# KillingSpark/zstd-rs

Hardware: AMD Instinct MI355X
Metric: decompressed_GB_per_s (higher is better)
Workload: dtype u8

## Files before the change

### zstd-rs_amd/csrc/zg_engine.cpp

```cpp
#include "zg_engine.h"
#include <stdlib.h>
#include <algorithm>
#include <string.h>

namespace zg {

#define ZG_HIP(call)                                  \
  do {                                                \
    hipError_t e_ = (call);                           \
    if (e_ != hipSuccess) return eng->fail(e_, #call); \
  } while (0)

#ifdef ZG_DEV_SWITCHES
static int g_poison = -1;
static uint64_t g_poisoned = 0;
uint64_t Poison::scratch_cap = 0;
int Poison::value() { return g_poison; }
void Poison::set(int v) { g_poison = v; }
void Poison::fill(void* p, size_t n, hipStream_t s) {
  if (g_poison < 0 || !p || !n) return;
  if (hipMemsetAsync(p, g_poison, n, s) == hipSuccess) g_poisoned += n;
}
void Poison::fill_now(void* p, size_t n) {
  if (g_poison < 0 || !p || !n) return;
// ... 28 lines not shown
}

int SidePass::reserve(size_t bytes) {
  const int st = buf.reserve(bytes);
  if (st) return st;
  Poison::fill_now(buf.p, buf.cap);
  for (hipEvent_t& e : ev) if (!e && hipEventCreate(&e) != hipSuccess) return ZG_HIP_ERROR;
  return 0;
}
hipError_t SidePass::upload(const void* a, size_t ab, const void* b, size_t bb, hipStream_t s) const {
  const hipError_t e = hipMemcpyAsync(buf.p, a, ab, hipMemcpyHostToDevice, s);
  return e != hipSuccess || !bb ? e : hipMemcpyAsync(at<uint8_t>(ab), b, bb, hipMemcpyHostToDevice, s);
}
hipError_t SidePass::end(hipStream_t s) const {
  const hipError_t e = hipGetLastError();
  return e != hipSuccess ? e : hipEventRecord(ev[1], s);
}
static hipError_t us_between(hipEvent_t a, hipEvent_t b, uint64_t* us) {
  float ms = 0;
  const hipError_t e = hipEventElapsedTime(&ms, a, b);
  if (e == hipSuccess) *us = (uint64_t)(ms * 1000.0f + 0.5f);
  return e;
}
hipError_t SidePass::elapsed_us(uint64_t* us) const { return us_between(ev[0], ev[1], us); }
void SidePass::release(int device) {
  if (buf.p && device >= 0) (void)hipSetDevice(device);
  buf.release();
  for (hipEvent_t& e : ev) if (e) { (void)hipEventDestroy(e); e = nullptr; }
  n = 0;
}

int Scratch::init_events() {
  if (have_events) return 0;
  for (auto& e : ev)
    if (hipEventCreate(&e) != hipSuccess) return ZG_HIP_ERROR;
  for (auto& e : ev_huf)
    if (hipEventCreate(&e) != hipSuccess) return ZG_HIP_ERROR;
  if (hipEventCreateWithFlags(&ev_fork, hipEventDisableTiming) != hipSuccess) return ZG_HIP_ERROR;
  if (hipEventCreateWithFlags(&ev_fork3, hipEventDisableTiming) != hipSuccess) return ZG_HIP_ERROR;
  if (hipEventCreateWithFlags(&ev_up, hipEventDisableTiming) != hipSuccess) return ZG_HIP_ERROR;
  for (auto& e : ev_sw)
    if (hipEventCreateWithFlags(&e, hipEventDisableTiming) != hipSuccess) return ZG_HIP_ERROR;
  for (auto& e : ev_flat)
    if (hipEventCreateWithFlags(&e, hipEventDisableTiming) != hipSuccess) return ZG_HIP_ERROR;
  have_events = true;
  return 0;
}
void Scratch::release_but_output() {
  DevBuf* all[] = {&d_src, &d_aux, &d_fparsed, &d_slot_log, &d_fse, &d_huf, &d_hufmax, &d_lit, &d_seq, &d_og, &d_raw};
  for (DevBuf* b : all) b->release();
}
template <class F> void Scratch::each_buf(F f) {
  DevBuf* all[] = {&d_src, &d_blocks, &d_frames, &d_aux, &d_fparsed, &d_slot_log, &d_fse, &d_huf, &d_hufmax, &d_status, &d_lit, &d_seq, &d_seqout, &d_pos,
                   &d_frameout, &d_dst, &d_seqblocks, &d_hufitems, &d_hufgroups, &d_totals, &d_og, &d_units, &d_unitinfo, &d_stepunits, &d_swdesc,
                   &d_dbg, &d_raw, &d_unitlist};
  for (DevBuf* b : all) f(*b);
}
void Scratch::release() {
  each_buf([](DevBuf& b) { b.release(); });
  for (auto& e : ev)
    if (e) { (void)hipEventDestroy(e); e = nullptr; }
  for (auto& e : ev_huf)
    if (e) { (void)hipEventDestroy(e); e = nullptr; }
  if (ev_fork) { (void)hipEventDestroy(ev_fork); ev_fork = nullptr; }
  if (ev_fork3) { (void)hipEventDestroy(ev_fork3); ev_fork3 = nullptr; }
  if (ev_up) { (void)hipEventDestroy(ev_up); ev_up = nullptr; }
  for (auto& e : ev_sw)
    if (e) { (void)hipEventDestroy(e); e = nullptr; }
  for (auto& e : ev_flat)
    if (e) { (void)hipEventDestroy(e); e = nullptr; }
  have_events = false;
}

int Engine::fail(hipError_t e, const char* what) {
  last_error = std::string(what) + ": " + hipGetErrorString(e);
  return ZG_HIP_ERROR;
}

Tuning Tuning::from_env() {
  Tuning t;
#ifdef ZG_DEV_SWITCHES
  t.dev_build = true;
  auto num = [](const char* name, uint32_t* v, bool positive) { const char* e = getenv(name); if (e && atoi(e) >= (positive ? 1 : 0)) *v = (uint32_t)atoi(e); return e != nullptr && atoi(e) >= 0; };
  auto is0 = [](const char* name) { const char* e = getenv(name); return e && e[0] == '0'; };
  num("ZGPU_UNIT_BLOCKS", &t.unit_blocks, true);
  t.direct = !is0("ZGPU_DIRECT");
  num("ZGPU_RAMP", &t.ramp_percent, false);
  t.sparse_set = num("ZGPU_SPARSE_MAX", &t.sparse_max, false);
  if (is0("ZGPU_LIT_DIRECT")) t.lit_direct = 0;
  else { const char* e = getenv("ZGPU_LIT_DIRECT"); if (e && e[0] == '1') t.lit_direct = 1; }
  { uint32_t v = 0; if (num("ZGPU_DIRECT_SHARE", &v, true) && v >= 10) t.direct_share10 = v; }
  t.debug_timers = getenv("ZGPU_DEBUG_TIMERS") != nullptr;
  { const char* e = getenv("ZGPU_FORCE_INORDER"); t.force_inorder = e && e[0] == '1'; }
  num("ZGPU_FLAT_MODE", &t.flat_mode, false);
  num("ZGPU_SWEEP_W", &t.sweep_w, true);
  t.overlap = !is0("ZGPU_OVERLAP");
  t.no_sweep = getenv("ZGPU_DEBUG_NO_SWEEP") != nullptr;
  t.sweep_split = !is0("ZGPU_SWEEP_SPLIT");
  t.no_exact = getenv("ZGPU_DEBUG_NO_EXACT") != nullptr;
  t.no_presize = is0("ZGPU_PRESIZE");
  { uint32_t v = 0; if (num("ZGPU_FLAT4", &v, false)) t.flat4 = (int)v; }
  { uint32_t v = 0; if (num("ZGPU_SEQ_PACKED", &v, false)) t.seq_packed = (int)v; }
  { const char* e = getenv("ZGPU_FLAT_T"); t.flat_shape = (e && atoi(e) == 512) ? 1 : 0; }
  num("ZGPU_SWEEP_MODE", &t.sweep.mode, false);
  num("ZGPU_SWEEP_NB", &t.sweep.nbatch, true);
  num("ZGPU_SWEEP_GROUP", &t.sweep.group, true);
  num("ZGPU_SWEEP_HEAD_LDS", &t.sweep.head_lds, false);
  num("ZGPU_SWEEP_HEAD_NB", &t.sweep.head_nbatch, true);
  { const char* e = getenv("ZGPU_FRAMES_SUBMIT_BYTES"); if (e && atoll(e) > 0) t.frames_submit_bytes = (uint64_t)atoll(e); }
  { const char* e = getenv("ZGPU_MEASURE_SUBMIT_BYTES"); if (e && atoll(e) > 0) t.measure_submit_bytes = (uint64_t)atoll(e); }
  num("ZGPU_SCATTER_CHUNK", &t.scatter_chunk, true);
  { const char* e = getenv("ZGPU_POISON"); if (e && e[0] && atoi(e) >= 0 && atoi(e) <= 255) t.poison = atoi(e); }
// ... 485 lines not shown
  b->bb.seq_packed_force = tn.seq_packed;
  if (tn.direct_share10) b->bb.direct_share10 = tn.direct_share10;
  b->bb.finish();
  BatchBuilder& bb = b->bb;
  Scratch* sc = b->sc = acquire();
  Poison::begin_submit();
  const uint32_t nb = (uint32_t)bb.blocks.size(), nf = (uint32_t)bb.frames.size();
  auto up = [&](DevBuf& d, const void* h, size_t bytes) -> int {
    int st = d.reserve(bytes ? bytes : 16);
    if (st) return st;
    Poison::fill(d.p, d.cap, us);
    if (bytes && hipMemcpyAsync(d.p, h, bytes, hipMemcpyHostToDevice, us) != hipSuccess) return ZG_HIP_ERROR;
    return 0;
  };
  int st = 0;
  if ((st = sc->d_src.reserve(len + 128))) { delete b; return st; }
  Poison::fill(sc->d_src.p, sc->d_src.cap, us);
  (void)hipMemsetAsync(sc->d_src.p, 0, 64, us);
  if (g) {
    const uint64_t at = (uint64_t)(uintptr_t)sc->d_src.p + 64;
    for (uint32_t j = 0; j < g->n; j++) {
      const DevEntry& en = g->e[g->idx[j]];
      if (en.len > len || g->off[j] > len - en.len) { delete b; return ZG_INTERNAL; }
      if (en.len) b->gather_segs_.push_back(zgs::Seg{en.src, at + g->off[j], en.len});
    }
    zgs::plan_chunks(b->gather_segs_.data(), (uint32_t)b->gather_segs_.size(), tn.scatter_chunk, &b->gather_chunks_);
    if (b->gather_chunks_.size() > 0xFFFFFFFFull) { delete b; return ZG_INTERNAL; }
    if (!b->gather_chunks_.empty()) {
      const size_t sb = b->gather_segs_.size() * sizeof(zgs::Seg), cb = b->gather_chunks_.size() * sizeof(zgs::Chunk);
      SidePass& p = b->side_[Batch::kSideGather];
      if ((st = p.reserve(sb + cb))) { delete b; return st; }
      bool ok = p.upload(b->gather_segs_.data(), sb, b->gather_chunks_.data(), cb, us) == hipSuccess && p.begin(us) == hipSuccess;
      if (ok) zg_launch_gather(p.at<zgs::Seg>(0), p.at<zgs::Chunk>(sb), (uint32_t)b->gather_chunks_.size(), us);
      ok = ok && p.end(us) == hipSuccess;
      if (!ok) { delete b; return ZG_HIP_ERROR; }
      b->gather_launched = true;
    }
  } else if (len && hipMemcpyAsync((uint8_t*)sc->d_src.p + 64, src, len, hipMemcpyHostToDevice, us) != hipSuccess) { delete b; return ZG_HIP_ERROR; }
  (void)hipMemsetAsync((uint8_t*)sc->d_src.p + 64 + len, 0, 64, us);
  const uint32_t nslots = bb.nslots();
  if ((st = up(sc->d_blocks, bb.blocks.data(), nb * sizeof(ZgBlock))) || (st = up(sc->d_frames, bb.frames.data(), nf * sizeof(ZgFrame))) ||
      (st = up(sc->d_seqblocks, bb.seq_blocks.data(), bb.seq_blocks.size() * 4)) ||
      (st = up(sc->d_hufitems, bb.huf_items.data(), bb.huf_items.size() * 4)) ||
      (st = up(sc->d_hufgroups, bb.huf_groups.data(), bb.huf_groups.size() * sizeof(ZgHufGroup))) ||
      (st = up(sc->d_units, bb.units.data(), bb.units.size() * sizeof(ZgUnit))) ||
      (st = up(sc->d_stepunits, bb.step_units.data(), bb.step_units.size() * 4)) ||
      (st = up(sc->d_unitlist, bb.unit_list.data(), bb.unit_list.size() * 4)) ||
      (st = sc->d_aux.reserve((size_t)nb * sizeof(ZgBlockAux) + 16)) || (st = sc->d_fparsed.reserve((size_t)nb * sizeof(ZgFtabParsed) + 16)) || (st = sc->d_slot_log.reserve((size_t)nslots * 4)) ||
      (st = sc->d_fse.reserve((size_t)nslots * ZG_FSE_SLOT_U32 * 4)) || (st = sc->d_huf.reserve((size_t)(bb.nhuf_slots + 1) * ZG_HUF_SLOT_U16 * 2)) ||
      (st = sc->d_hufmax.reserve(bb.nhuf_slots + 16)) || (st = sc->d_status.reserve(7 * ((size_t)nb * 4 + 16))) ||
      (st = sc->d_lit.reserve(bb.lit_bytes + 128)) || (st = sc->d_seq.reserve((bb.seq_count + 2) * sizeof(ZgSeq))) ||
      (st = sc->d_raw.reserve((bb.seq_count + 8) * 4)) ||
      (st = sc->d_seqout.reserve((size_t)nb * sizeof(ZgBlockSeqOut) + 16)) || (st = sc->d_pos.reserve((size_t)nb * sizeof(ZgBlockPos) + 16)) ||
      (st = sc->d_frameout.reserve((size_t)nf * sizeof(ZgFrameOut) + 16)) || (st = sc->d_totals.reserve(64)) ||
      (st = sc->d_swdesc.reserve(bb.step_units.size() * sizeof(ZgSweepDesc) + 32)) ||
      (st = sc->d_unitinfo.reserve(bb.units.size() * sizeof(ZgUnitInfo) + 16)) || (st = sc->d_dbg.reserve(8192)) || (st = sc->init_events())) {
    delete b;
    return st;
  }
  if (Poison::value() >= 0) {
    DevBuf* up_bufs[] = {&sc->d_src, &sc->d_blocks, &sc->d_frames, &sc->d_seqblocks, &sc->d_hufitems, &sc->d_hufgroups, &sc->d_units, &sc->d_stepunits, &sc->d_unitlist};
    sc->each_buf([&](DevBuf& x) {
      bool uploaded = false;
      for (DevBuf* u : up_bufs) uploaded = uploaded || u == &x;
      if (!uploaded) Poison::fill(x.p, x.cap, us);
    });
#ifdef ZG_DEV_SWITCHES
    Poison::scratch_cap = 0;
    sc->each_buf([&](DevBuf& x) { Poison::scratch_cap += x.p ? x.cap : 0; });
#endif
  }
  ZgBatchDev& d = b->dev;
  d.src = sc->d_src.as<uint8_t>() + 64; d.src_len = len;
  d.blocks = sc->d_blocks.as<ZgBlock>(); d.nblocks = nb;
  d.frames = sc->d_frames.as<ZgFrame>(); d.nframes = nf;
  d.nslots = nslots; d.nhuf_slots = bb.nhuf_slots;
  d.aux = sc->d_aux.as<ZgBlockAux>(); d.ftab_parsed = sc->d_fparsed.as<ZgFtabParsed>(); d.slot_log = sc->d_slot_log.as<uint8_t>();
  d.fse_arena = sc->d_fse.as<uint32_t>(); d.huf_arena = sc->d_huf.as<uint16_t>(); d.huf_maxbits = sc->d_hufmax.as<uint8_t>();
  d.status = sc->d_status.as<uint32_t>(); d.tab_status = d.status + nb + 4; d.lit_status = d.tab_status + nb + 4;
  d.lit_counts = d.lit_status + nb + 4;
  d.lit_arena = sc->d_lit.as<uint8_t>() + 64;
  d.seq_arena = sc->d_seq.as<ZgSeq>(); d.raw_arena = sc->d_raw.as<uint32_t>();
  d.seq_out = sc->d_seqout.as<ZgBlockSeqOut>(); d.pos = sc->d_pos.as<ZgBlockPos>(); d.frame_out = sc->d_frameout.as<ZgFrameOut>();
  d.dst = nullptr; d.dst_cap = 0; d.og = nullptr;
  d.dict = nullptr;
  d.seq_blocks = sc->d_seqblocks.as<uint32_t>(); d.nseq_blocks = (uint32_t)bb.seq_blocks.size();
  d.huf_items = sc->d_hufitems.as<uint32_t>(); d.huf_groups = sc->d_hufgroups.as<ZgHufGroup>(); d.nhuf_groups = (uint32_t)bb.huf_groups.size();
  d.totals = sc->d_totals.as<uint32_t>();
  d.units = sc->d_units.as<ZgUnit>(); d.nunits = (uint32_t)bb.units.size(); d.unit_info = sc->d_unitinfo.as<ZgUnitInfo>();
  d.step_units = sc->d_stepunits.as<uint32_t>();
  d.unit_list = sc->d_unitlist.as<uint32_t>(); d.ndirect = bb.n_direct;
  d.sweep_desc = sc->d_swdesc.as<ZgSweepDesc>();
  b->sweep_steps.clear();
  for (const ZgStepRange& r : bb.steps) {
    ZgSweepStep ss;
    ss.list_off = r.list_off; ss.nunits = r.nunits; ss.slices = r.max_blocks * (kMaxBlockSize / ZG_SW_BATCH); ss.pad = 0;
    b->sweep_steps.push_back(ss);
  }
  d.dbg = tn.debug_timers ? sc->d_dbg.as<unsigned long long>() : nullptr;
  d.flags = tn.force_inorder ? 1u : 0u;
  d.flags |= (uint32_t)flat_shape_ << 2;
  d.flags |= ((tn.flat_mode & 3u) << 4) | ((tn.flat_mode & 4u) << 5);
  d.sweep_window = tn.sweep_w;
  if (side) {
    if (hipEventRecord(sc->ev_up, us) != hipSuccess) { delete b; return ZG_HIP_ERROR; }
    b->wait_upload = true;
  } else if (hipStreamSynchronize(stream_) != hipSuccess) { delete b; return ZG_HIP_ERROR; }
  if (b->gather_launched && !side && b->side_[Batch::kSideGather].elapsed_us(&b->gather_us) != hipSuccess) { delete b; return ZG_HIP_ERROR; }
  *out = b;
  return ZG_OK;
}

int Batch::run() {
  ZG_HIP(hipSetDevice(eng->device_));
  hipStream_t s = eng->stream_;
  ZgBatchDev& d = dev;
  if (d.nframes == 0) { ran = true; total_out = 0; return ZG_OK; }
  if (d.nblocks == 0) {
    frame_out.assign(d.nframes, ZgFrameOut{});
    for (ZgFrameOut& fo : frame_out) fo.err_packed = 0xFFFFFFFFu;
    total_out = 0; ran = false; synced = true;
    return ZG_OK;
  }
  hipEvent_t* ev = sc->ev;
  presized = false;
  d.dst_cap_pre = 0;
  dictfill_launches = 0; dictfill_bytes = 0; dictfill_us = 0; side_[kSideFill0].n = side_[kSideFill1].n = 0;
  if (!fs && all_declared && declared_total && !eng->no_presize_ && declared_total <= bb.out_bound && !bb.ramped && frame_dicts_.empty()) {
    if (sc->d_og.reserve(declared_total * 4 + 64) == 0 && sc->d_dst.reserve(kOutFront + declared_total + 64) == 0) {
      Poison::fill(sc->d_og.p, sc->d_og.cap, s); Poison::fill(sc->d_dst.p, sc->d_dst.cap, s);
      d.dst = sc->d_dst.as<uint8_t>() + kOutFront; d.dst_cap = declared_total;
      d.og = sc->d_og.as<uint32_t>(); d.og_words = og_words = declared_total;
      d.dst_cap_pre = declared_total;
      presized = true;
    } else { sc->d_og.release(); sc->d_dst.release(); }
  }
  if (wait_upload) { ZG_HIP(hipStreamWaitEvent(s, sc->ev_up, 0)); wait_upload = false; }
  ZG_HIP(hipEventRecord(ev[0], s));
  if (fs) {
    ZgFrame& fr0 = bb.frames[0];
    fr0.hist_init[0] = fs->hist[0]; fr0.hist_init[1] = fs->hist[1]; fr0.hist_init[2] = fs->hist[2];
// ... 158 lines not shown
  } else {
    if ((st = sc->d_dst.reserve(kOutFront + total_out + 64))) return st;
    Poison::fill(sc->d_dst.p, sc->d_dst.cap, s);
    d.dst = sc->d_dst.as<uint8_t>() + kOutFront; d.dst_cap = total_out;
    og_words = total_out;
  }
  if (any_fast && (st = sc->d_og.reserve(og_words * 4 + 64))) return st;
  Poison::fill(sc->d_og.p, sc->d_og.cap, s);
  d.og = sc->d_og.as<uint32_t>();
  d.og_words = og_words;
  return ZG_OK;
}

int Batch::launch_phase2() {
  hipStream_t s = eng->stream_;
  ZgBatchDev& d = dev;
  hipEvent_t* ev = sc->ev;
  if (bb.lit_direct) {
    d.flags |= ZG_FLAG_LIT_DIRECT;
    ZG_HIP(hipEventRecord(sc->ev_huf[0], s));
    zg_launch_huf(d, s);
    zg_launch_litfix(d, s);
    ZG_HIP(hipEventRecord(sc->ev_huf[1], s));
  }
  zg_launch_lit(d, s);
  ZG_HIP(hipEventRecord(ev[6], s));
  sweep_mode = 0; synced = false;
  int flat4 = eng->tn_.flat4;
  if (flat4 < 0) {
    const uint32_t cus = (uint32_t)eng->cus_, nd = d.ndirect;
    flat4 = nd >= 16u * cus ? 6 : nd >= 8u * cus ? 4 : nd >= 4u * cus ? 1 : 0;
  }
  const bool overlap = bb.ramped && eng->tn_.overlap && !eng->tn_.no_sweep;
  d.overlap_epoch = overlap ? ++epoch_ : 0u;
  if (overlap) {
    hipStream_t s3 = eng->stream3_;
    ZG_HIP(hipMemsetAsync(d.unit_info, 0, (size_t)d.nunits * sizeof(ZgUnitInfo), s));
    ZG_HIP(hipEventRecord(sc->ev_fork3, s));
    zg_launch_flat(d, s, eng->stream2_, sc->ev_flat, flat4);
    ZG_HIP(hipEventRecord(ev[7], s));
    ZG_HIP(hipStreamWaitEvent(s3, sc->ev_fork3, 0));
    launch_sweep(true, s3);
    ZG_HIP(hipEventRecord(sc->ev_fork3, s3));
    ZG_HIP(hipStreamWaitEvent(s, sc->ev_fork3, 0));
  } else {
    zg_launch_flat(d, s, eng->stream2_, sc->ev_flat, flat4);
    { bool any = false; for (const ZgFrame& fr : bb.frames) any = any || fr.sparse; if (any) zg_launch_sparse(d, s); }
    ZG_HIP(hipEventRecord(ev[7], s));
    if (!eng->tn_.no_sweep) launch_sweep(true);
  }
  ZG_HIP(hipEventRecord(ev[8], s));
  zg_launch_lz(d, s);
  ZG_HIP(hipEventRecord(ev[9], s));
  return ZG_OK;
}

void Batch::launch_sweep(bool split, hipStream_t main) {
  if (!main) main = eng->stream_;
  if (!eng->tn_.sweep_split) split = false;
  uint64_t wmax = 0, wmin = ~0ull;
  for (const ZgFrame& fr : bb.frames) {
    wmax = fr.window_size > wmax ? fr.window_size : wmax;
    wmin = fr.window_size < wmin ? fr.window_size : wmin;
    if (fr.hist_init[0] != 1 || fr.hist_init[1] != 4 || fr.hist_init[2] != 8 || fr.dict_len || fr.prior_out) split = false;
  }
  if (dev.sweep_window) wmax = wmin = dev.sweep_window;
  if (wmax > 0x7FFFFFFFull) wmax = 0x7FFFFFFFull;
  if (wmin > wmax) wmin = wmax;
  split_sweep = zg_launch_sweep(dev, main, sweep_steps.data(), (uint32_t)sweep_steps.size(), eng->stream2_, sc->ev_sw, split ? 80u : 0u,
                                bb.unit_blocks_used * kMaxBlockSize, (uint32_t)wmax, (uint32_t)wmin, eng->tn_.sweep);
  sweep_mode = split_sweep ? 1u : sweep_mode;
}

void Batch::release_scratch() {
  if (!sc || !eng || !synced) return;
  (void)hipSetDevice(eng->device_);
  sc->release_but_output();
  dev.og = nullptr; dev.src = nullptr; dev.lit_arena = nullptr; dev.seq_arena = nullptr; dev.raw_arena = nullptr;
  ran = false;
}

int Batch::sync() {
  ZG_HIP(hipSetDevice(eng->device_));
  ZG_HIP(hipStreamSynchronize(eng->stream_));
  if (dev.nframes == 0 || !ran) return ZG_OK;
  if (presized) {
    uint32_t totals[4] = {0, 0, 0, 0};
    ZG_HIP(hipMemcpy(totals, dev.totals, 16, hipMemcpyDeviceToHost));
    total_out = (uint64_t)totals[0] | ((uint64_t)totals[1] << 32);
    far_seen = totals[3] != 0;
    frame_out.resize(dev.nframes);
    if (totals[2]) {
      presized = false;
      dev.dst_cap_pre = 0;
      uint32_t zero = 0;
      ZG_HIP(hipMemcpy(dev.totals + 2, &zero, 4, hipMemcpyHostToDevice));
      int st = size_output();
      if (!st) st = launch_phase2();
      if (st) return st;
      ZG_HIP(hipStreamSynchronize(eng->stream_));
    }
  }
  if (split_sweep) {
    uint32_t far = 0;
    ZG_HIP(hipMemcpy(&far, dev.totals + 3, 4, hipMemcpyDeviceToHost));
    if (far) {
      launch_sweep(false);
      ZG_HIP(hipStreamSynchronize(eng->stream_));
      sweep_mode = 2;
    }
    split_sweep = false;
  }
  ZG_HIP(hipMemcpy(frame_out.data(), dev.frame_out, (size_t)dev.nframes * sizeof(ZgFrameOut), hipMemcpyDeviceToHost));
  {
    bool need = far_seen;
    for (uint32_t f = 0; f < dev.nframes && !need; f++) {
      const ZgFrame& fr = bb.frames[f];
      const uint32_t st = frame_out[f].status;
      need = st == (uint32_t)ZG_EXE_OFFSET_TOO_BIG || st == (uint32_t)ZG_EXE_DICT_TOO_SMALL || fr.dict_len != 0 ||
             st == (uint32_t)ZG_EXE_NOT_ENOUGH_LITERALS || st == (uint32_t)ZG_EXE_ZERO_OFFSET ||
             fr.hist_init[0] > fr.window_size || fr.hist_init[1] > fr.window_size || fr.hist_init[2] > fr.window_size;
    }
    if (need && !eng->tn_.no_exact) {
      zg_launch_exact(dev, eng->stream_, drain_rule);
      ZG_HIP(hipStreamSynchronize(eng->stream_));
      ZG_HIP(hipMemcpy(frame_out.data(), dev.frame_out, (size_t)dev.nframes * sizeof(ZgFrameOut), hipMemcpyDeviceToHost));
      exact_ran = true;
    }
  }
  {
    uint32_t nfail = 0;
    for (uint32_t f = 0; f < dev.nframes; f++) nfail += frame_out[f].status && frame_out[f].good_blocks < bb.frames[f].nblocks;
    std::vector<ZgBlockPos> all_pos;
    if (nfail > 8) { all_pos.resize(dev.nblocks); ZG_HIP(hipMemcpy(all_pos.data(), dev.pos, (size_t)dev.nblocks * sizeof(ZgBlockPos), hipMemcpyDeviceToHost)); }
    for (uint32_t f = 0; f < dev.nframes && nfail; f++) {
      ZgFrameOut& fo = frame_out[f];
      const ZgFrame& fr = bb.frames[f];
      if (!fo.status || fo.good_blocks >= fr.nblocks) continue;
      ZgBlockPos p;
      if (!all_pos.empty()) p = all_pos[fr.first_block + fo.good_blocks];
      else ZG_HIP(hipMemcpy(&p, dev.pos + fr.first_block + fo.good_blocks, sizeof p, hipMemcpyDeviceToHost));
      if (p.out_base < fo.out_size) fo.out_size = p.out_base;
    }
  }
  if (fs && dev.nframes == 1 && !frame_out.empty()) {
    ZgFrameOut& fo = frame_out[0];
    const ZgFrame& fr = bb.frames[0];
    const uint32_t st = fo.status;
    const bool exe = st == (uint32_t)ZG_EXE_NOT_ENOUGH_LITERALS || st == (uint32_t)ZG_EXE_ZERO_OFFSET || st == (uint32_t)ZG_EXE_OFFSET_TOO_BIG ||
                     st == (uint32_t)ZG_EXE_DICT_TOO_SMALL;
    if (exe && fo.good_blocks < fr.nblocks) {
      const uint32_t b = fr.first_block + fo.good_blocks;
      const ZgBlock& blk = bb.blocks[b];
      ZgBlockSeqOut so;
      memset(&so, 0, sizeof so);
      if (blk.btype == ZG_BT_COMPRESSED && blk.nseq && !blk.host_status)
        ZG_HIP(hipMemcpy(&so, dev.seq_out + b, sizeof so, hipMemcpyDeviceToHost));
      if (so.pad && so.pad <= blk.nseq) {
        const uint32_t j = so.pad - 1u;
        const bool lits = st != (uint32_t)ZG_EXE_NOT_ENOUGH_LITERALS;
        const uint64_t used = kOutFront + fs->base + fs->have + fo.out_size;
        const uint64_t room = fs->d_out.cap > used + 64 ? fs->d_out.cap - used - 64 : 0;
        const uint32_t limit = room > 0xFFFFFF00ull ? 0xFFFFFF00u : (uint32_t)room;
        zg_launch_partial(dev, eng->stream_, 0, b, j, lits, limit);
        ZG_HIP(hipStreamSynchronize(eng->stream_));
        uint32_t psize = 0;
// ... 347 lines not shown
```

### zstd-rs_amd/csrc/zg_engine.h

```cpp
#pragma once
#include <hip/hip_runtime.h>
#include <stddef.h>
#include <stdint.h>
#include <string>
#include <vector>
#include "zg_host_parse.h"
#include "zg_kernels.h"

namespace zg {

constexpr size_t kOutFront = 256;

struct Poison {
#ifdef ZG_DEV_SWITCHES
  static int value();
  static void set(int v);
  static void fill(void* p, size_t n, hipStream_t s);
  static void fill_now(void* p, size_t n);
  static void begin_submit();
  static uint64_t bytes();
  static uint64_t scratch_cap;
#else
  static int value() { return -1; }
  static void fill(void*, size_t, hipStream_t) {}
// ... 5 lines not shown

struct DevBuf {
  void* p = nullptr;
  size_t cap = 0;
  int reserve(size_t n, bool keep = false, hipStream_t s = nullptr);
  void release();
  template <typename T> T* as() const { return (T*)p; }
};

struct SidePass {
  DevBuf buf;
  hipEvent_t ev[2] = {nullptr, nullptr};
  uint32_t n = 0;
  size_t back = 0;
  int reserve(size_t bytes);
  hipError_t upload(const void* a, size_t ab, const void* b, size_t bb, hipStream_t s) const;
  hipError_t begin(hipStream_t s) const { return hipEventRecord(ev[0], s); }
  hipError_t end(hipStream_t s) const;
  hipError_t elapsed_us(uint64_t* us) const;
  void release(int device = -1);
  template <typename T> T* at(size_t off) const { return (T*)((uint8_t*)buf.p + off); }
};

struct FrameState {
  DevBuf d_out;
  uint64_t base = 0;
  uint64_t have = 0;
  uint64_t produced = 0;
  uint32_t hist[3] = {1, 4, 8};
  uint64_t counted = 0;
  DevBuf d_fse;
  DevBuf d_huf;
  DevBuf d_tmp;
  uint8_t logs[4] = {0, 0, 0, 0};
  uint8_t huf_maxbits = 0;
  uint32_t carry_mask = 0;
  uint64_t window_size = 0;
  uint8_t* out_ptr() const { return (uint8_t*)d_out.p + kOutFront; }
  int make_room(uint64_t extra, uint64_t keep, hipStream_t s);
  int reserve_window(uint64_t payload, hipStream_t s);
  bool room_moves(uint64_t extra, uint64_t keep) const {
    if (keep > have) keep = have;
    if (base && keep < have && d_out.p) return true;
    return !d_out.p || kOutFront + base + have + extra + 64 > d_out.cap;
  }
  void reset();
  void release();
};

enum { ZG_T_TABLES = 0, ZG_T_HUF, ZG_T_SEQ, ZG_T_SEQPOST, ZG_T_SCAN, ZG_T_LIT, ZG_T_FLAT, ZG_T_SWEEP, ZG_T_LZ, ZG_T_TOTAL, ZG_T_COUNT };

struct Scratch {
  DevBuf d_src, d_blocks, d_frames, d_aux, d_fparsed, d_slot_log, d_fse, d_huf, d_hufmax, d_status, d_lit, d_seq, d_seqout, d_pos, d_frameout,
      d_dst, d_seqblocks, d_hufitems, d_hufgroups, d_totals, d_og, d_units, d_unitinfo, d_stepunits, d_swdesc, d_dbg, d_raw, d_unitlist;
  hipEvent_t ev[ZG_T_COUNT + 1] = {};
  hipEvent_t ev_up = nullptr;
  hipEvent_t ev_huf[2] = {}, ev_fork = nullptr, ev_fork3 = nullptr;
  hipEvent_t ev_sw[80] = {};
  hipEvent_t ev_flat[2] = {};
  bool have_events = false;
  template <class F> void each_buf(F f);
  int init_events();
  void release();
  void release_but_output();
};

struct Tuning {
  bool dev_build = false;
  uint32_t unit_blocks = 0;
  bool direct = true;
  uint32_t ramp_percent = 0;
  bool sparse_set = false;
  uint32_t sparse_max = 0;
  int lit_direct = -1;
  uint32_t direct_share10 = 0;
  bool debug_timers = false;
  bool force_inorder = false;
  uint32_t flat_mode = 0;
  uint32_t sweep_w = 0;
  bool overlap = true;
  bool no_sweep = false;
  bool sweep_split = true;
  bool no_exact = false;
  bool no_presize = false;
  int flat4 = -1;
  int flat_shape = 0;
  int seq_packed = -1;
  ZgSweepTuning sweep;
  uint64_t measure_submit_bytes = 0;
  uint64_t frames_submit_bytes = 0;
  uint32_t scatter_chunk = 0;
  bool hash_device_max_set = false;
  uint64_t hash_device_max = 0;
  int poison = -1;
  static Tuning from_env();
};

class Engine;

enum { kPassLaunches = 0, kPassUs = 1, kPassBytes = 2 };

class Batch {
 public:
  ~Batch();
  BatchBuilder bb;
  std::vector<FrameInfo> info;
  std::vector<ZgFrameOut> frame_out;
// ... 140 lines not shown
```

### zstd-rs_amd/csrc/zg_kernels.hip

```cpp
#include <stdlib.h>
#include "zg_kernels.h"
#include "zg_dev.h"
#include "zg_xxh64_dev.h"
#include "zg_scatter.h"

#define ZG_SEQ_G 16
#define ZG_LZ_T 256

typedef uint32_t zg_v4u __attribute__((ext_vector_type(4)));
typedef __attribute__((address_space(1))) zg_v4u zg_gv4u;
typedef uint32_t zg_v2u __attribute__((ext_vector_type(2)));
typedef __attribute__((address_space(1))) zg_v2u zg_gv2u;
typedef uint32_t zg_v3u __attribute__((ext_vector_type(3)));
typedef __attribute__((address_space(1))) zg_v3u zg_gv3u;
__device__ __forceinline__ uint32_t zg_ld32_fun(const uint8_t* p) {
  const uint64_t a = (uint64_t)p;
  const zg_v2u v = *(const zg_gv2u*)(a & ~3ull);
  return __builtin_amdgcn_alignbit(v.y, v.x, ((uint32_t)a & 3u) * 8u);
}

__device__ __forceinline__ void zg_set_status(uint32_t* status, uint32_t b, int st) {
  if (st) atomicCAS(&status[b], 0u, (uint32_t)st);
}
__device__ __forceinline__ uint32_t zg_sweep_window(const ZgBatchDev& d, const ZgFrame& fr) {
// ... 511 lines not shown
  const uint32_t a0 = zg_bfi(up, c.w2, c.w0), a1 = zg_bfi(up, c.w3, c.w1), a2 = zg_bfi(up, c.w3, c.w2);
  const uint32_t d0 = zg_bfi(odd, a1, a0), d1 = zg_bfi(odd, a2, a1);
  const uint32_t bits = __builtin_amdgcn_ubfe(__builtin_amdgcn_alignbit(d1, d0, rel), 0u, nb);
  const uint32_t st2 = PK ? ((c.e & 0x3FFu) >> 1) + bits - ((1u << nb0) >> 1) : (c.e >> 4) + bits;
  if (FAST) {
    const uint32_t st = c.st;
    c.st = st2;
    c.e = ZG_SEQ_LD16(tab, st2); if (!PK) c.s = ZG_SEQ_LD8(xtab, st2);
    __builtin_amdgcn_sched_barrier(0);
    c.pr -= (int32_t)tot;
    zg_seq_window(c, store4);
    *rec = (uint16_t)st;
    __builtin_amdgcn_sched_barrier(0);
  } else {
    const int32_t q = c.pr - (int32_t)tot;
    const bool ok = act && q >= rbits;
    rec[cnt * 4u] = (uint16_t)c.st;
    cnt += ok ? 1u : 0u;
    const bool was = act;
    left -= ok ? 1u : 0u;
    act = ok && left != 0u;
    ZgSeqChain n = c;
    n.pr = q; n.st = st2; n.e = ZG_SEQ_LD16(tab, st2); if (!PK) n.s = ZG_SEQ_LD8(xtab, st2);
    zg_seq_window(n, store4);
    __builtin_amdgcn_sched_barrier(0);
    if (was) { c.pr = n.pr; c.r0 = n.r0; c.w0 = n.w0; c.w1 = n.w1; c.w2 = n.w2; c.w3 = n.w3; }
    if (act) { c.st = n.st; c.e = n.e; c.s = n.s; }
  }
}

template <bool PK>
__global__ void __launch_bounds__(128) zg_k_seq(ZgBatchDev d) {
#ifdef ZG_SEQ_ILV
  __shared__ __attribute__((aligned(16))) uint8_t s_tabi[((ZG_FSE_SLOT_U32 + 2) * 2 + 15) / 16 * 256];
  __shared__ __attribute__((aligned(16))) uint8_t s_xbi[PK ? 16 : (ZG_FSE_SLOT_U32 + 4 + 15) / 16 * 256];
#define ZG_SEQ_ST16(g, i, v) (*(uint16_t*)(s_tabi + (ZG_SEQ_ILVA(2u * (i)) | ((g) << 4))) = (v))
#define ZG_SEQ_ST8(g, i, v) (s_xbi[ZG_SEQ_ILVA((uint32_t)(i)) | ((g) << 4)] = (v))
#else
  __shared__ uint16_t s_tab[ZG_SEQ_G][ZG_FSE_SLOT_U32 + 2];
  __shared__ uint8_t s_xb[PK ? 1 : ZG_SEQ_G][PK ? 4 : ZG_FSE_SLOT_U32 + 4];
#define ZG_SEQ_ST16(g, i, v) (s_tab[g][i] = (v))
#define ZG_SEQ_ST8(g, i, v) (s_xb[g][i] = (v))
#endif
  __shared__ __attribute__((aligned(16))) uint8_t s_ring[ZG_SEQ_G][ZG_SEQ_RSTORE];
  __shared__ __attribute__((aligned(16))) uint2 s_out[2][ZG_SEQ_G][ZG_SEQ_CH];
  __shared__ int32_t s_pos[2][ZG_SEQ_G];
  __shared__ uint32_t s_cnt[2][ZG_SEQ_G];
  __shared__ uint32_t s_more[2];
  __shared__ uint64_t s_fetch_hi[ZG_SEQ_G], s_fetch_lo[ZG_SEQ_G];
  __shared__ uint8_t s_log[ZG_SEQ_G][4];
  __shared__ int s_ok[ZG_SEQ_G];
  const uint32_t base = blockIdx.x * ZG_SEQ_G, t = threadIdx.x;
  const bool mover = t >= 64u;
  for (uint32_t g = 0; g < ZG_SEQ_G; g++) {
    uint32_t idx = base + g;
    if (idx >= d.nseq_blocks) break;
    uint32_t b = d.seq_blocks[idx];
    const ZgBlock* blk = &d.blocks[b];
    int32_t sl[3] = {blk->ll_slot, blk->of_slot, blk->ml_slot};
    const uint32_t offs[3] = {ZG_FSE_LL_OFF, ZG_FSE_OF_OFF, ZG_FSE_ML_OFF};
    bool ok = d.status[b] == 0;
    for (int k = 0; k < 3; k++) {
      if (sl[k] < 0) { ok = false; continue; }
      if ((uint32_t)sl[k] < d.nblocks && d.status[sl[k]] != 0) { ok = false; continue; }
      unsigned lg = d.slot_log[(uint64_t)sl[k] * 4 + k];
      if (lg > 9) { ok = false; continue; }
      const uint32_t* g_t = d.fse_arena + (uint64_t)sl[k] * ZG_FSE_SLOT_U32 + offs[k];
      {
        uint32_t v[4];
#pragma unroll
        for (int j = 0; j < 4; j++) { const uint32_t i = t + 128 * j; v[j] = i < (1u << lg) ? g_t[i] : 0u; }
#pragma unroll
        for (int j = 0; j < 4; j++) {
          const uint32_t i = t + 128 * j;
          if (i < (1u << lg)) {
            const uint32_t nb = ZG_FSE_NB(v[j]);
            const uint32_t all = nb + (k == 1 ? ZG_FSE_SYM(v[j]) : v[j] >> 26);
            if (PK) ZG_SEQ_ST16(g, offs[k] + i, ZG_SEQ_PK(ZG_FSE_BL(v[j]), nb, all));
            else { ZG_SEQ_ST16(g, offs[k] + i, (uint16_t)((ZG_FSE_BL(v[j]) << 4) | nb)); ZG_SEQ_ST8(g, offs[k] + i, (uint8_t)all); }
          }
        }
      }
      if (t == 0) s_log[g][k] = (uint8_t)lg;
    }
    if (t == 0) { s_ok[g] = ok ? 1 : 0; ZG_SEQ_ST16(g, ZG_FSE_SLOT_U32, PK ? ZG_SEQ_PK(0, 0, 0) : 0); if (!PK) ZG_SEQ_ST8(g, ZG_FSE_SLOT_U32, 0); }
  }
  __syncthreads();
  const uint32_t g = (t & 63u) >> 2, role = t & 3u;
  const bool owner = role == 3u;
  bool act = base + g < d.nseq_blocks;
  bool have = false;
  uint32_t b = 0, nseq = 0, left = 0;
  int32_t rbits = 0;
  uint64_t bsA = 0, floorA = 0, lo = 0, dstp = 0;
  const uint32_t toff = role == 0u ? ZG_FSE_OF_OFF : role == 1u ? ZG_FSE_ML_OFF : role == 2u ? ZG_FSE_LL_OFF : ZG_FSE_SLOT_U32;
#ifdef ZG_SEQ_ILV
  const uint16_t* tab = (const uint16_t*)(s_tabi + (g << 4));
  const uint8_t* xtab = PK ? s_xbi : s_xbi + (g << 4);
  const uint32_t to2 = toff * 2u, to1 = toff;
#else
  const uint16_t* tab = &s_tab[g][toff];
  const uint8_t* xtab = PK ? &s_xb[0][0] : &s_xb[g][toff];
  const uint32_t to2 = 0, to1 = 0;
#endif
  uint8_t* const store = s_ring[g];
  const uint8_t* const store4 = store + 4;
  int32_t P = 0;
  int status = ZG_OK;
  if (act) {
    b = d.seq_blocks[base + g];
    const ZgBlock blk = d.blocks[b];
    if (!s_ok[g]) {
      const uint32_t bo = d.aux[b].seq_bits_off;
      const bool nopad = bo <= blk.src_len && (blk.src_len == bo || d.src[blk.src_off + blk.src_len - 1u] == 0);
      if (owner && !mover) zg_set_status(d.status, b, nopad ? ZG_SEQ_EXTRA_PADDING : ZG_FSE_UNINIT);
      act = false;
    } else {
      const uint32_t bits_off = d.aux[b].seq_bits_off;
      if (bits_off > blk.src_len) { if (owner && !mover) zg_set_status(d.status, b, ZG_INTERNAL); act = false; }
      else {
        const uint8_t* bs = d.src + blk.src_off + bits_off;
        const uint32_t bs_len = blk.src_len - bits_off;
        nseq = blk.nseq;
        const uint32_t lastb = bs_len ? bs[bs_len - 1] : 0;
        if (bs_len == 0 || lastb == 0) { if (owner && !mover) zg_set_status(d.status, b, ZG_SEQ_EXTRA_PADDING); act = false; }
        else {
          P = (int32_t)(bs_len - 1) * 8 + (int32_t)(zg_hbit(lastb) - 1);
          bsA = (uint64_t)bs;
          rbits = (int32_t)((uint32_t)(bsA & (ZG_SEQ_RING - 1)) * 8u);
          floorA = (bsA & ~15ull) - 16;
          dstp = (uint64_t)(d.raw_arena + blk.seq_base);
          have = true;
        }
      }
    }
  }
  {
    uint64_t top = 0, want = 0;
    if (act) {
      top = (bsA + (uint64_t)(P >> 3) + 8 + 15) & ~15ull;
      const uint64_t p0 = bsA + (uint64_t)(P >> 3);
      want = p0 > ZG_SEQ_MARGIN + 16 ? (p0 - ZG_SEQ_MARGIN - 16) & ~15ull : 0;
      if (want < floorA) want = floorA;
      lo = want;
    }
    if (owner && !mover) { s_fetch_hi[g] = act ? top : 0; s_fetch_lo[g] = act ? want : 0; }
    __syncthreads();
    for (uint32_t j = t; j < ZG_SEQ_G * ZG_SEQ_PRO; j += 128) {
      const uint32_t gg = j / ZG_SEQ_PRO, k = j % ZG_SEQ_PRO;
      const uint64_t hi = s_fetch_hi[gg], addr = hi - 16ull * (k + 1);
      if (hi && addr >= s_fetch_lo[gg] && addr < hi) { const zg_v4u v = *(const zg_gv4u*)addr; zg_ring_put(s_ring[gg], addr, v); }
    }
    __syncthreads();
  }
  ZgSeqChain c = {0, 0, 0, 0, 0, 0, 0, 0, 0};
  if (act) {
    const uint32_t ll_log = s_log[g][0], of_log = s_log[g][1], ml_log = s_log[g][2];
    const uint32_t lg = role == 0u ? of_log : role == 1u ? ml_log : role == 2u ? ll_log : 0u;
    const int32_t q = P - (int32_t)(role == 2u ? ll_log : role == 0u ? ll_log + of_log : ll_log + of_log + ml_log);
    c.st = (q >= 0 && role != 3u) ? zg_ring_bits(store, q + rbits, lg) : 0u;
    c.e = ZG_SEQ_LD16(tab, c.st); c.s = PK ? 0u : ZG_SEQ_LD8(xtab, c.st);
    P -= (int32_t)(ll_log + of_log + ml_log);
    if (owner && !mover) d.seq_out[b].pad = (uint32_t)P;
    left = nseq;
  }
  c.pr = P + rbits;
#ifdef ZG_PROFILE_SEQ
  unsigned long long tcs[3] = {0, 0, 0}, tl_ = clock64();
#define ZG_QTICK(i) { const unsigned long long n_ = clock64(); tcs[i] += n_ - tl_; tl_ = n_; }
#else
#define ZG_QTICK(i)
#endif
  if (!mover) {
    if (act) zg_seq_window(c, store4);
    for (uint32_t par = 0;; par ^= 1u) {
      uint16_t* const out_base = (uint16_t*)&s_out[par][g][0] + role;
      uint32_t cnt = 0;
      if (act && left > ZG_SEQ_CH) {
#pragma unroll
        for (int k = 0; k < ZG_SEQ_CH; k++) zg_seq_step<true, PK>(c, tab, xtab, store4, out_base + 4 * k, rbits, act, left, cnt, to2, to1);
        cnt = ZG_SEQ_CH; left -= ZG_SEQ_CH;
        if (c.pr < rbits) act = false;
      } else if (act) {
#pragma unroll
        for (int k = 0; k < ZG_SEQ_CH; k++) zg_seq_step<false, PK>(c, tab, xtab, store4, out_base, rbits, act, left, cnt, to2, to1);
      }
      P = c.pr - rbits;
      const bool more = __any(act);
      if (owner) { s_pos[par][g] = P; s_cnt[par][g] = cnt | (act ? 256u : 0u); }
      if (t == 0) s_more[par] = more ? 1u : 0u;
      ZG_QTICK(0)
      __syncthreads();
      ZG_QTICK(1)
      if (!more) break;
    }
    if (have && owner) {
      if (left != 0) status = ZG_SEQ_NOT_ENOUGH_BYTES;
      else if (P > 0) status = ZG_SEQ_EXTRA_BITS;
      zg_set_status(d.status, b, status);
    }
  } else {
    zg_v4u piece[ZG_SEQ_PREG];
    uint64_t piece_addr[ZG_SEQ_PREG];
    bool piece_ok[ZG_SEQ_PREG];
#pragma unroll
    for (int pi = 0; pi < ZG_SEQ_PREG; pi++) { piece[pi] = zg_v4u{0, 0, 0, 0}; piece_addr[pi] = 0; piece_ok[pi] = false; }
    for (uint32_t par = 0;; par ^= 1u) {
      __syncthreads();
      const uint32_t cw = s_cnt[par][g], cnt = cw & 255u;
      const bool live = have && (cw >> 8) != 0u;
      const int32_t pos = s_pos[par][g];
      const bool more = s_more[par] != 0u;
      zg_v2u rec[(ZG_SEQ_CH + 3) / 4];
#pragma unroll
      for (int i = 0; i < (ZG_SEQ_CH + 3) / 4; i++) rec[i] = *(const zg_v2u*)&s_out[par][g][role + 4u * (uint32_t)i];
#pragma unroll
      for (int pi = 0; pi < ZG_SEQ_PREG; pi++) if (piece_ok[pi]) zg_ring_put(store, piece_addr[pi], piece[pi]);
      {
        uint64_t hi = 0, want = 0;
        if (live) {
          const uint64_t p0 = bsA + (uint64_t)(pos >> 3);
          want = p0 > ZG_SEQ_MARGIN ? (p0 - ZG_SEQ_MARGIN) & ~15ull : 0;
          if (want < floorA) want = floorA;
          if (want < lo) { hi = lo; lo = want; }
        }
#pragma unroll
        for (int pi = 0; pi < ZG_SEQ_PREG; pi++) {
          const uint64_t addr = hi - 16ull * (role + 4u * (uint32_t)pi + 1u);
          piece_ok[pi] = hi && addr >= want && addr < hi;
          if (piece_ok[pi]) { piece[pi] = *(const zg_gv4u*)addr; piece_addr[pi] = addr; }
        }
      }
#pragma unroll
      for (int i = 0; i < (ZG_SEQ_CH + 3) / 4; i++) {
        const uint32_t k = role + 4u * (uint32_t)i;
        if (k < cnt) ((__attribute__((address_space(1))) uint32_t*)dstp)[k] = ZG_RAW_PACK(rec[i].x & 0xFFu, (rec[i].x >> 16) & 0x1FFu, rec[i].y & 0x1FFu);
      }
      dstp += (uint64_t)cnt * 4u;
      if (!more) break;
    }
  }
#ifdef ZG_PROFILE_SEQ
  if (t == 0 && d.dbg) { atomicAdd(&d.dbg[16], tcs[0]); atomicAdd(&d.dbg[17], tcs[1]); atomicAdd(&d.dbg[18], 1ull); }
#endif
#undef ZG_QTICK
}

#define ZG_SP_T 256
#define ZG_SP_S 8
template <int S> __device__ __forceinline__ void zg_map_scan_step(ZgHistMap& m, uint32_t lane) {
  ZgHistMap pm;
  pm.s[0] = zx_scan_src<S>(m.s[0], 1u << 30); pm.s[1] = zx_scan_src<S>(m.s[1], 2u << 30); pm.s[2] = zx_scan_src<S>(m.s[2], 3u << 30);
  if (zx_scan_takes<S>(lane)) m = zg_map_compose(pm, m);
}
__device__ __forceinline__ ZgHistMap zg_map_scan_incl(ZgHistMap m, uint32_t lane) {
  zg_map_scan_step<0>(m, lane); zg_map_scan_step<1>(m, lane); zg_map_scan_step<2>(m, lane); zg_map_scan_step<3>(m, lane);
  zg_map_scan_step<4>(m, lane); zg_map_scan_step<5>(m, lane);
  return m;
}
__device__ __forceinline__ ZgHistMap zg_map_shr1(const ZgHistMap& m) {
  ZgHistMap r;
  r.s[0] = zx_shr1(m.s[0], 1u << 30); r.s[1] = zx_shr1(m.s[1], 2u << 30); r.s[2] = zx_shr1(m.s[2], 3u << 30);
  return r;
}
__global__ void __launch_bounds__(ZG_SP_T, 4) zg_k_seqpost(ZgBatchDev d) {
  __shared__ ZgHistMap s_wm[ZG_SP_T / 64];
  __shared__ uint32_t s_wl[ZG_SP_T / 64], s_wo[ZG_SP_T / 64], s_wx[ZG_SP_T / 64];
  __shared__ uint32_t s_err;
  __shared__ uint32_t s_llb[36], s_mlb[53];
  __shared__ uint16_t s_t[ZG_FSE_SLOT_U32];
  __shared__ uint32_t s_tr[ZG_SP_T / 64][64 * 25];
  const uint32_t t = threadIdx.x, lane = t & 63, wv = t >> 6;
  const uint32_t b = d.seq_blocks[blockIdx.x];
  if (d.status[b]) return;
  const ZgBlock blk = d.blocks[b];
  {
    const int32_t sl[3] = {blk.ll_slot, blk.ml_slot, blk.of_slot};
    const uint32_t offs[4] = {ZG_FSE_LL_OFF, ZG_FSE_ML_OFF, ZG_FSE_OF_OFF, ZG_FSE_SLOT_U32};
#pragma unroll
    for (int k = 0; k < 3; k++) {
      const uint32_t* g_t = d.fse_arena + (uint64_t)sl[k] * ZG_FSE_SLOT_U32;
      for (uint32_t i = offs[k] + t; i < offs[k + 1]; i += ZG_SP_T) { const uint32_t v = g_t[i]; s_t[i] = (uint16_t)((ZG_FSE_SYM(v) << 4) | ZG_FSE_NB(v)); }
    }
  }
  const uint32_t nseq = blk.nseq, regen = blk.regen_size;
  const uint32_t wlim = zg_sweep_window(d, d.frames[blk.frame]);
  const uint8_t* bs = d.src + blk.src_off + d.aux[b].seq_bits_off;
  const uint32_t* raw = d.raw_arena + blk.seq_base;
  ZgSeq* out = d.seq_arena + blk.seq_base;
  if (t == 0) s_err = 0xFFFFFFFFu;
  if (t < 36) s_llb[t] = ZG_LL_BASE[t] | ((uint32_t)ZG_LL_BITS[t] << 24);
  if (t < 53) s_mlb[t] = ZG_ML_BASE[t] | ((uint32_t)ZG_ML_BITS[t] << 24);
  ZgHistMap carry = zg_map_identity();
  uint32_t lit_carry = 0, out_carry = 0;
  uint32_t pos_carry = d.seq_out[b].pad;
  uint32_t err_i0 = 0;
// ... 1053 lines not shown
```

Baseline: 111.8.

## Batch end-of-run readback into pinned buffer and parallelize sequence-kernel table prologue

The totals and frame_out results are packed into one device buffer and copied asynchronously into a pinned host buffer at the end of the launch. This replaces up to three separate blocking hipMemcpy calls after the stream sync with plain host memcpy. Separately, the sequence kernel prologue no longer loops serially over 16 groups to load the FSE tables. Table descriptors are computed in parallel into shared memory, then 8 threads per group load all three tables concurrently, and per-block metadata is prefetched early. The cost is an extra pinned allocation, and the readback must fall back to hipMemcpy when a second sweep makes the cached data stale.

Result: no change. 112.7, median of 6 (+0.8%).

```diff
diff --git a/zstd-rs_amd/csrc/zg_engine.cpp b/zstd-rs_amd/csrc/zg_engine.cpp
--- a/zstd-rs_amd/csrc/zg_engine.cpp
+++ b/zstd-rs_amd/csrc/zg_engine.cpp
@@ -104,12 +104,21 @@
 }
 template <class F> void Scratch::each_buf(F f) {
   DevBuf* all[] = {&d_src, &d_blocks, &d_frames, &d_aux, &d_fparsed, &d_slot_log, &d_fse, &d_huf, &d_hufmax, &d_status, &d_lit, &d_seq, &d_seqout, &d_pos,
-                   &d_frameout, &d_dst, &d_seqblocks, &d_hufitems, &d_hufgroups, &d_totals, &d_og, &d_units, &d_unitinfo, &d_stepunits, &d_swdesc,
+                   &d_frameout, &d_dst, &d_seqblocks, &d_hufitems, &d_hufgroups, &d_og, &d_units, &d_unitinfo, &d_stepunits, &d_swdesc,
                    &d_dbg, &d_raw, &d_unitlist};
   for (DevBuf* b : all) f(*b);
 }
+int Scratch::reserve_end(size_t bytes) {
+  if (h_end && bytes <= h_end_cap) return 0;
+  if (h_end) { (void)hipHostFree(h_end); h_end = nullptr; h_end_cap = 0; }
+  const size_t ncap = bytes < 4096 ? 4096 : bytes;
+  if (hipHostMalloc(&h_end, ncap, hipHostMallocDefault) != hipSuccess) { (void)hipGetLastError(); h_end = nullptr; return ZG_NOMEM; }
+  h_end_cap = ncap;
+  return 0;
+}
 void Scratch::release() {
   each_buf([](DevBuf& b) { b.release(); });
+  if (h_end) { (void)hipHostFree(h_end); h_end = nullptr; h_end_cap = 0; }
   for (auto& e : ev)
     if (e) { (void)hipEventDestroy(e); e = nullptr; }
   for (auto& e : ev_huf)
@@ -701,7 +710,8 @@
       (st = sc->d_lit.reserve(bb.lit_bytes + 128)) || (st = sc->d_seq.reserve((bb.seq_count + 2) * sizeof(ZgSeq))) ||
       (st = sc->d_raw.reserve((bb.seq_count + 8) * 4)) ||
       (st = sc->d_seqout.reserve((size_t)nb * sizeof(ZgBlockSeqOut) + 16)) || (st = sc->d_pos.reserve((size_t)nb * sizeof(ZgBlockPos) + 16)) ||
-      (st = sc->d_frameout.reserve((size_t)nf * sizeof(ZgFrameOut) + 16)) || (st = sc->d_totals.reserve(64)) ||
+      (st = sc->d_frameout.reserve(Scratch::kEndHead + (size_t)nf * sizeof(ZgFrameOut) + 16)) ||
+      (st = sc->reserve_end(Scratch::kEndHead + (size_t)nf * sizeof(ZgFrameOut))) ||
       (st = sc->d_swdesc.reserve(bb.step_units.size() * sizeof(ZgSweepDesc) + 32)) ||
       (st = sc->d_unitinfo.reserve(bb.units.size() * sizeof(ZgUnitInfo) + 16)) || (st = sc->d_dbg.reserve(8192)) || (st = sc->init_events())) {
     delete b;
@@ -730,12 +740,12 @@
   d.lit_counts = d.lit_status + nb + 4;
   d.lit_arena = sc->d_lit.as<uint8_t>() + 64;
   d.seq_arena = sc->d_seq.as<ZgSeq>(); d.raw_arena = sc->d_raw.as<uint32_t>();
-  d.seq_out = sc->d_seqout.as<ZgBlockSeqOut>(); d.pos = sc->d_pos.as<ZgBlockPos>(); d.frame_out = sc->d_frameout.as<ZgFrameOut>();
+  d.seq_out = sc->d_seqout.as<ZgBlockSeqOut>(); d.pos = sc->d_pos.as<ZgBlockPos>(); d.frame_out = (ZgFrameOut*)(sc->d_frameout.as<uint8_t>() + Scratch::kEndHead);
   d.dst = nullptr; d.dst_cap = 0; d.og = nullptr;
   d.dict = nullptr;
   d.seq_blocks = sc->d_seqblocks.as<uint32_t>(); d.nseq_blocks = (uint32_t)bb.seq_blocks.size();
   d.huf_items = sc->d_hufitems.as<uint32_t>(); d.huf_groups = sc->d_hufgroups.as<ZgHufGroup>(); d.nhuf_groups = (uint32_t)bb.huf_groups.size();
-  d.totals = sc->d_totals.as<uint32_t>();
+  d.totals = sc->d_frameout.as<uint32_t>();
   d.units = sc->d_units.as<ZgUnit>(); d.nunits = (uint32_t)bb.units.size(); d.unit_info = sc->d_unitinfo.as<ZgUnitInfo>();
   d.step_units = sc->d_stepunits.as<uint32_t>();
   d.unit_list = sc->d_unitlist.as<uint32_t>(); d.ndirect = bb.n_direct;
@@ -1000,6 +1010,7 @@
   ZG_HIP(hipEventRecord(ev[8], s));
   zg_launch_lz(d, s);
   ZG_HIP(hipEventRecord(ev[9], s));
+  ZG_HIP(hipMemcpyAsync(sc->h_end, d.totals, Scratch::kEndHead + (size_t)d.nframes * sizeof(ZgFrameOut), hipMemcpyDeviceToHost, s));
   return ZG_OK;
 }
 
@@ -1032,9 +1043,11 @@
   ZG_HIP(hipSetDevice(eng->device_));
   ZG_HIP(hipStreamSynchronize(eng->stream_));
   if (dev.nframes == 0 || !ran) return ZG_OK;
+  const uint8_t* const h_end = (const uint8_t*)sc->h_end;
+  bool end_fresh = true;
   if (presized) {
     uint32_t totals[4] = {0, 0, 0, 0};
-    ZG_HIP(hipMemcpy(totals, dev.totals, 16, hipMemcpyDeviceToHost));
+    memcpy(totals, h_end, 16);
     total_out = (uint64_t)totals[0] | ((uint64_t)totals[1] << 32);
     far_seen = totals[3] != 0;
     frame_out.resize(dev.nframes);
@@ -1051,15 +1064,18 @@
   }
   if (split_sweep) {
     uint32_t far = 0;
-    ZG_HIP(hipMemcpy(&far, dev.totals + 3, 4, hipMemcpyDeviceToHost));
+    memcpy(&far, h_end + 12, 4);
     if (far) {
       launch_sweep(false);
       ZG_HIP(hipStreamSynchronize(eng->stream_));
       sweep_mode = 2;
+      end_fresh = false;
     }
     split_sweep = false;
   }
-  ZG_HIP(hipMemcpy(frame_out.data(), dev.frame_out, (size_t)dev.nframes * sizeof(ZgFrameOut), hipMemcpyDeviceToHost));
+  frame_out.resize(dev.nframes);
+  if (end_fresh) memcpy(frame_out.data(), h_end + Scratch::kEndHead, (size_t)dev.nframes * sizeof(ZgFrameOut));
+  else ZG_HIP(hipMemcpy(frame_out.data(), dev.frame_out, (size_t)dev.nframes * sizeof(ZgFrameOut), hipMemcpyDeviceToHost));
   {
     bool need = far_seen;
     for (uint32_t f = 0; f < dev.nframes && !need; f++) {
diff --git a/zstd-rs_amd/csrc/zg_engine.h b/zstd-rs_amd/csrc/zg_engine.h
--- a/zstd-rs_amd/csrc/zg_engine.h
+++ b/zstd-rs_amd/csrc/zg_engine.h
@@ -81,7 +81,11 @@
 
 struct Scratch {
   DevBuf d_src, d_blocks, d_frames, d_aux, d_fparsed, d_slot_log, d_fse, d_huf, d_hufmax, d_status, d_lit, d_seq, d_seqout, d_pos, d_frameout,
-      d_dst, d_seqblocks, d_hufitems, d_hufgroups, d_totals, d_og, d_units, d_unitinfo, d_stepunits, d_swdesc, d_dbg, d_raw, d_unitlist;
+      d_dst, d_seqblocks, d_hufitems, d_hufgroups, d_og, d_units, d_unitinfo, d_stepunits, d_swdesc, d_dbg, d_raw, d_unitlist;
+  static constexpr size_t kEndHead = 128;
+  void* h_end = nullptr;
+  size_t h_end_cap = 0;
+  int reserve_end(size_t bytes);
   hipEvent_t ev[ZG_T_COUNT + 1] = {};
   hipEvent_t ev_up = nullptr;
   hipEvent_t ev_huf[2] = {}, ev_fork = nullptr, ev_fork3 = nullptr;
diff --git a/zstd-rs_amd/csrc/zg_kernels.hip b/zstd-rs_amd/csrc/zg_kernels.hip
--- a/zstd-rs_amd/csrc/zg_kernels.hip
+++ b/zstd-rs_amd/csrc/zg_kernels.hip
@@ -587,45 +587,83 @@
   __shared__ int s_ok[ZG_SEQ_G];
   const uint32_t base = blockIdx.x * ZG_SEQ_G, t = threadIdx.x;
   const bool mover = t >= 64u;
-  for (uint32_t g = 0; g < ZG_SEQ_G; g++) {
-    uint32_t idx = base + g;
-    if (idx >= d.nseq_blocks) break;
-    uint32_t b = d.seq_blocks[idx];
-    const ZgBlock* blk = &d.blocks[b];
-    int32_t sl[3] = {blk->ll_slot, blk->of_slot, blk->ml_slot};
-    const uint32_t offs[3] = {ZG_FSE_LL_OFF, ZG_FSE_OF_OFF, ZG_FSE_ML_OFF};
-    bool ok = d.status[b] == 0;
-    for (int k = 0; k < 3; k++) {
-      if (sl[k] < 0) { ok = false; continue; }
-      if ((uint32_t)sl[k] < d.nblocks && d.status[sl[k]] != 0) { ok = false; continue; }
-      unsigned lg = d.slot_log[(uint64_t)sl[k] * 4 + k];
-      if (lg > 9) { ok = false; continue; }
-      const uint32_t* g_t = d.fse_arena + (uint64_t)sl[k] * ZG_FSE_SLOT_U32 + offs[k];
-      {
-        uint32_t v[4];
-#pragma unroll
-        for (int j = 0; j < 4; j++) { const uint32_t i = t + 128 * j; v[j] = i < (1u << lg) ? g_t[i] : 0u; }
-#pragma unroll
-        for (int j = 0; j < 4; j++) {
-          const uint32_t i = t + 128 * j;
-          if (i < (1u << lg)) {
-            const uint32_t nb = ZG_FSE_NB(v[j]);
-            const uint32_t all = nb + (k == 1 ? ZG_FSE_SYM(v[j]) : v[j] >> 26);
-            if (PK) ZG_SEQ_ST16(g, offs[k] + i, ZG_SEQ_PK(ZG_FSE_BL(v[j]), nb, all));
-            else { ZG_SEQ_ST16(g, offs[k] + i, (uint16_t)((ZG_FSE_BL(v[j]) << 4) | nb)); ZG_SEQ_ST8(g, offs[k] + i, (uint8_t)all); }
-          }
-        }
-      }
-      if (t == 0) s_log[g][k] = (uint8_t)lg;
-    }
-    if (t == 0) { s_ok[g] = ok ? 1 : 0; ZG_SEQ_ST16(g, ZG_FSE_SLOT_U32, PK ? ZG_SEQ_PK(0, 0, 0) : 0); if (!PK) ZG_SEQ_ST8(g, ZG_FSE_SLOT_U32, 0); }
-  }
-  __syncthreads();
+#ifdef ZG_PROFILE_SEQ
+  const unsigned long long tp0_ = clock64();
+#endif
   const uint32_t g = (t & 63u) >> 2, role = t & 3u;
   const bool owner = role == 3u;
   bool act = base + g < d.nseq_blocks;
+  uint32_t b = 0, f_bits_off = 0, f_lastb = 0;
+  ZgBlock blk;
+  blk.src_off = 0; blk.src_len = 0; blk.nseq = 0; blk.seq_base = 0;
+  if (act) {
+    b = d.seq_blocks[base + g];
+    blk = d.blocks[b];
+    f_bits_off = d.aux[b].seq_bits_off;
+    f_lastb = f_bits_off < blk.src_len ? d.src[blk.src_off + blk.src_len - 1u] : 0u;
+  }
+  uint64_t* const s_desc = (uint64_t*)&s_out[0][0][0];
+  static_assert(sizeof(uint2) * 2 * ZG_SEQ_G * ZG_SEQ_CH >= 8 * 3 * ZG_SEQ_G, "48 table descriptors in the records' buffers");
+  if (t < 3u * ZG_SEQ_G) {
+    const uint32_t dg = t / 3u, k = t % 3u, idx = base + dg;
+    uint64_t desc = 0;
+    uint32_t lg = 0;
+    if (idx < d.nseq_blocks) {
+      const uint32_t db = d.seq_blocks[idx];
+      const ZgBlock* dblk = &d.blocks[db];
+      const int32_t sl = k == 0u ? dblk->ll_slot : k == 1u ? dblk->of_slot : dblk->ml_slot;
+      const uint32_t bst = d.status[db];
+      if (sl >= 0) {
+        const uint32_t dst = (uint32_t)sl < d.nblocks ? d.status[sl] : 0u;
+        lg = d.slot_log[(uint64_t)sl * 4 + k];
+        const uint32_t off = k == 0u ? ZG_FSE_LL_OFF : k == 1u ? ZG_FSE_OF_OFF : ZG_FSE_ML_OFF;
+        if (bst == 0u && dst == 0u && lg <= 9u) desc = (1ull << 63) | ((uint64_t)lg << 56) | ((uint64_t)sl * ZG_FSE_SLOT_U32 + off);
+        else lg = 0;
+      }
+    }
+    s_desc[t] = desc;
+    s_log[dg][k] = (uint8_t)lg;
+  }
+  __syncthreads();
+  {
+    const uint32_t tg = t >> 3, l8 = t & 7u;
+    const uint32_t offs[3] = {ZG_FSE_LL_OFF, ZG_FSE_OF_OFF, ZG_FSE_ML_OFF};
+    uint32_t n[3];
+    const uint32_t* g_t[3];
+#pragma unroll
+    for (int k = 0; k < 3; k++) {
+      const uint64_t dk = s_desc[3u * tg + (uint32_t)k];
+      n[k] = (dk >> 63) ? 1u << ((uint32_t)(dk >> 56) & 15u) : 0u;
+      g_t[k] = d.fse_arena + (dk & 0x00FFFFFFFFFFFFFFull);
+    }
+    if (l8 == 0u) {
+      s_ok[tg] = (n[0] && n[1] && n[2]) ? 1 : 0;
+      ZG_SEQ_ST16(tg, ZG_FSE_SLOT_U32, PK ? ZG_SEQ_PK(0, 0, 0) : 0); if (!PK) ZG_SEQ_ST8(tg, ZG_FSE_SLOT_U32, 0);
+    }
+    const uint32_t n01 = n[0] > n[1] ? n[0] : n[1], nmax = n01 > n[2] ? n01 : n[2];
+    for (uint32_t i0 = l8; i0 < nmax; i0 += 64u) {
+      uint32_t v[3][8];
+#pragma unroll
+      for (int k = 0; k < 3; k++)
+#pragma unroll
+        for (int j = 0; j < 8; j++) { const uint32_t i = i0 + 8u * (uint32_t)j; v[k][j] = i < n[k] ? g_t[k][i] : 0u; }
+#pragma unroll
+      for (int k = 0; k < 3; k++)
+#pragma unroll
+        for (int j = 0; j < 8; j++) {
+          const uint32_t i = i0 + 8u * (uint32_t)j;
+          if (i < n[k]) {
+            const uint32_t nb = ZG_FSE_NB(v[k][j]);
+            const uint32_t all = nb + (k == 1 ? ZG_FSE_SYM(v[k][j]) : v[k][j] >> 26);
+            if (PK) ZG_SEQ_ST16(tg, offs[k] + i, ZG_SEQ_PK(ZG_FSE_BL(v[k][j]), nb, all));
+            else { ZG_SEQ_ST16(tg, offs[k] + i, (uint16_t)((ZG_FSE_BL(v[k][j]) << 4) | nb)); ZG_SEQ_ST8(tg, offs[k] + i, (uint8_t)all); }
+          }
+        }
+    }
+  }
+  __syncthreads();
   bool have = false;
-  uint32_t b = 0, nseq = 0, left = 0;
+  uint32_t nseq = 0, left = 0;
   int32_t rbits = 0;
   uint64_t bsA = 0, floorA = 0, lo = 0, dstp = 0;
   const uint32_t toff = role == 0u ? ZG_FSE_OF_OFF : role == 1u ? ZG_FSE_ML_OFF : role == 2u ? ZG_FSE_LL_OFF : ZG_FSE_SLOT_U32;
@@ -643,21 +681,19 @@
   int32_t P = 0;
   int status = ZG_OK;
   if (act) {
-    b = d.seq_blocks[base + g];
-    const ZgBlock blk = d.blocks[b];
     if (!s_ok[g]) {
-      const uint32_t bo = d.aux[b].seq_bits_off;
-      const bool nopad = bo <= blk.src_len && (blk.src_len == bo || d.src[blk.src_off + blk.src_len - 1u] == 0);
+      const uint32_t bo = f_bits_off;
+      const bool nopad = bo <= blk.src_len && (blk.src_len == bo || f_lastb == 0);
       if (owner && !mover) zg_set_status(d.status, b, nopad ? ZG_SEQ_EXTRA_PADDING : ZG_FSE_UNINIT);
       act = false;
     } else {
-      const uint32_t bits_off = d.aux[b].seq_bits_off;
+      const uint32_t bits_off = f_bits_off;
       if (bits_off > blk.src_len) { if (owner && !mover) zg_set_status(d.status, b, ZG_INTERNAL); act = false; }
       else {
         const uint8_t* bs = d.src + blk.src_off + bits_off;
         const uint32_t bs_len = blk.src_len - bits_off;
         nseq = blk.nseq;
-        const uint32_t lastb = bs_len ? bs[bs_len - 1] : 0;
+        const uint32_t lastb = bs_len ? f_lastb : 0;
         if (bs_len == 0 || lastb == 0) { if (owner && !mover) zg_set_status(d.status, b, ZG_SEQ_EXTRA_PADDING); act = false; }
         else {
           P = (int32_t)(bs_len - 1) * 8 + (int32_t)(zg_hbit(lastb) - 1);
@@ -702,6 +738,7 @@
   c.pr = P + rbits;
 #ifdef ZG_PROFILE_SEQ
   unsigned long long tcs[3] = {0, 0, 0}, tl_ = clock64();
+  const unsigned long long tpro_ = tl_ - tp0_;
 #define ZG_QTICK(i) { const unsigned long long n_ = clock64(); tcs[i] += n_ - tl_; tl_ = n_; }
 #else
 #define ZG_QTICK(i)
@@ -776,7 +813,7 @@
     }
   }
 #ifdef ZG_PROFILE_SEQ
-  if (t == 0 && d.dbg) { atomicAdd(&d.dbg[16], tcs[0]); atomicAdd(&d.dbg[17], tcs[1]); atomicAdd(&d.dbg[18], 1ull); }
+  if (t == 0 && d.dbg) { atomicAdd(&d.dbg[16], tcs[0]); atomicAdd(&d.dbg[17], tcs[1]); atomicAdd(&d.dbg[18], 1ull); atomicAdd(&d.dbg[19], tpro_); }
 #endif
 #undef ZG_QTICK
 }
```
